# ohsnyt/bzip2-rust

Hardware: AMD Instinct MI355X
Metric: compress MB/s at -9 (900 KB blocks), 1/2/4/8 MI355X; bit-exact vs C bzip2 (higher is better)
Workload: dtype u8; 1 GPU; 1024 MiB per GPU synthetic text at -9 (1194 blocks on this rank), BASELINE configs[2]; raw_bytes_total=1073741824, blocks_rank0=1194, compressed_bytes=323302688

## Files before the change

### bzip2-rust_amd/csrc/bzx_bsort.hip

```cpp
#include <hip/hip_runtime.h>
#include "bzx_host.h"
#include "bzx_wg.h"
#include "bzx_pack.h"

#define BS_NT 1024
#define BS_NW (BS_NT / 64)
#ifndef BS_C
#define BS_C 2048
#endif
#define BS_FW (BS_C / 64)
#define BS_ISO (BS_C / 3)
#ifndef BS_ISO_SHIFT
#define BS_ISO_SHIFT 5
#endif
#ifndef BS_BIN1
#define BS_BIN1 15
#endif
#define BS_BIN2 12
#define BS_NBIN1 (1u << BS_BIN1)
#define BS_TAB_WORDS (BS_NBIN1 + (BS_NBIN1 >> 5))
#define BS_MAX_BK 1024
#ifndef BS_MAX_BIG
#define BS_MAX_BIG 512
#endif
// ... 425 lines not shown
            uint32_t pv[SP_V];
            auto load_tile = [&](uint32_t t0) {
#pragma unroll
                for (uint32_t u = 0; u < SP_V; u++) {
                    const uint32_t i0 = t0 + (u * BS_NT + tid) * 4;
                    hi[u] = lo[u] = 0;
                    pv[u] = 0;
                    if (i0 < n) {
                        uint64_t w2[2];
                        __builtin_memcpy(w2, P + ((i0 * bits) >> 3), 16);
                        hi[u] = w2[0];
                        lo[u] = w2[1];
                        if (i0 >= 1 && i0 + 3 <= n) {
                            __builtin_memcpy(&pv[u], T + i0 - 1, 4);
                        } else {
                            const uint32_t nvalid = n - i0 < 4u ? n - i0 : 4u;
                            for (uint32_t e = 0; e < nvalid; e++) pv[u] |= (uint32_t)T[i0 + e ? i0 + e - 1 : n - 1] << (8 * e);
                        }
                    }
                }
            };
            load_tile(0);
            bzx_lds_barrier();
            uint32_t tpar = 0;
            for (uint32_t t0 = 0; t0 < n; t0 += SP_TILE, tpar ^= 1u) {
                uint32_t *tcnt = tpar ? tcnt1 : tcnt0, *tother = tpar ? tcnt0 : tcnt1;
                uint32_t kr[SP_V * 4], key[SP_V * 4], pvc[SP_V];
#pragma unroll
                for (uint32_t u = 0; u < SP_V; u++) {
                    const uint32_t i0 = t0 + (u * BS_NT + tid) * 4;
                    const uint32_t nvalid = i0 < n ? (n - i0 < 4u ? n - i0 : 4u) : 0u;
                    const uint32_t sh0 = (i0 * bits) & 7u;
                    const uint64_t h = __builtin_bswap64(hi[u]), l = __builtin_bswap64(lo[u]);
                    pvc[u] = pv[u];
#pragma unroll
                    for (uint32_t e = 0; e < 4; e++) {
                        kr[u * 4 + e] = 0xFFFFFFFFu;
                        key[u * 4 + e] = 0;
                        if (e < nvalid) {
                            const uint32_t sh = sh0 + e * bits;
                            const uint64_t w = sh ? (h << sh) | (l >> (64u - sh)) : h;
                            const uint32_t kb = tab16[(uint32_t)(w >> (64 - BS_BIN1))], k = kb & 1023u;
                            key[u * 4 + e] = (uint32_t)((w << (kb >> 10)) >> 32);
                            kr[u * 4 + e] = k | (atomicAdd(&tcnt[k], 1u) << 16);
                        }
                    }
                }
                if (t0 + SP_TILE < n) load_tile(t0 + SP_TILE);
                bzx_lds_barrier();
                {
                    const uint32_t c = tid < nbk ? tcnt[tid] : 0u;
                    const uint32_t incl = bzx_wave_incl_sum(c);
                    uint32_t *wtot = b_scratch + tpar * BS_NW;
                    if (bzx_lane() == 63) wtot[bzx_wave()] = incl;
                    bzx_lds_barrier();
                    uint32_t pre = 0;
                    const uint32_t wv = bzx_wave();
#pragma unroll
                    for (uint32_t i = 0; i < BS_NW; i++) pre += i < wv ? wtot[i] : 0u;
                    const uint32_t ex = pre + incl - c;
                    if (tid < nbk) {
                        tcnt[tid] = ex;
                        tother[tid] = 0;
                        delta[tid] = b_start[tid] + b_cur[tid] - ex;
                        b_cur[tid] += c;
                    }
                }
                bzx_lds_barrier();
#pragma unroll
                for (uint32_t u = 0; u < SP_V; u++)
#pragma unroll
                    for (uint32_t e = 0; e < 4; e++)
                        if (kr[u * 4 + e] != 0xFFFFFFFFu) {
                            const uint32_t k = kr[u * 4 + e] & 0xFFFFu, rel = (u * BS_NT + tid) * 4 + e;
                            stage[tcnt[k] + (kr[u * 4 + e] >> 16)] = ((uint64_t)key[u * 4 + e] << 32) | ((uint64_t)k << 21) | ((uint64_t)rel << 8) |
                                                                     (uint64_t)((pvc[u] >> (8 * e)) & 255u);
                        }
                bzx_lds_barrier();
                const uint32_t tn = n - t0 < SP_TILE ? n - t0 : SP_TILE;
#pragma unroll
                for (uint32_t u = 0; u < SP_TILE / BS_NT; u++) {
                    const uint32_t i = u * BS_NT + tid;
                    if (i < tn) {
                        const uint64_t r = stage[i];
                        const uint32_t k = (uint32_t)(r >> 21) & 1023u, rel = (uint32_t)(r >> 8) & 8191u;
                        rec_a[delta[k] + i] = (r & 0xFFFFFFFF00000000ull) | ((uint64_t)(t0 + rel) << 12) | ((r & 255ull) << 4);
                    }
                }
            }
        }
        __syncthreads();
        DIAG_STAMP(101);
        bool ok = bucket_emit<BS_BIN1>(B, b, j_, nbk, 0, 0, 0, bits, 0, 0);
        DIAG_STAMP(102);

        if (ok) ok = deep_process(B, b, j_, n, bits, P, rec_a, rec_b, 0, 0, BZX_DEEP_LEVELS > 0 ? 0 : -1);
        DIAG_STAMP(103);
        if (!ok) DIAG_COUNT(107, 1);
        if (!ok && tid == 0) block_redo(B, b);
        __syncthreads();
    }
    DIAG_FLUSH();
}

__global__ __launch_bounds__(BS_NT) void bzx_bsplit_deep_kernel(BzxBatch B)
{
    const uint32_t tid = threadIdx.x, lvl = B.deep_lvl;
    const uint32_t listed = B.counters[BZX_CTR_DEEP_CNT + lvl];
    const uint32_t n_items = listed < B.deep_cap ? listed : B.deep_cap;
    if (n_items == 0) return;
    DIAG_T0();
    const BzxDeepItem *list = reinterpret_cast<const BzxDeepItem *>(B.deep_list) + (size_t)(lvl & 1u) * B.deep_cap;
    for (;;) {
        if (tid == 0) b_bcast[0] = atomicAdd(&B.counters[BZX_CTR_DEEP_FETCH + lvl], 1u);
        __syncthreads();
        const uint32_t i = b_bcast[0];
        __syncthreads();
        if (i >= n_items) break;
        const BzxDeepItem d = list[i];
        if (d.cnt == 0) continue;
        const uint32_t b = d.blk;
        if (__atomic_load_n(&B.blk[b].status, __ATOMIC_RELAXED) & BZX_ST_REDO) continue;
        const uint32_t n = B.blk[b].n, bits = d.dbits >> 16;
        const size_t sb = BZX_SLAB(B, b);
        const uint8_t *__restrict__ P = B.pk + sb * BZX_PK_STRIDE;
        uint64_t *__restrict__ rec_a = B.rec_a + sb * BZX_MAX_N;
        uint64_t *__restrict__ rec_b = B.rec_b + sb * BZX_MAX_N;
        if (tid == 0) {
            b_bcast[3] = 1;
            b_bcast[4] = 0;
            b_big[0][0] = d.st;
            b_big[0][1] = d.cnt;
            b_big[0][2] = d.dbits & 0xFFFFu;
        }
        __syncthreads();
        const bool ok = deep_process(B, b, (b - B.blk_first) / B.blk_step, n, bits, P, rec_a, rec_b, 0, 1,
                                     lvl + 1 < BZX_DEEP_LEVELS ? (int)lvl + 1 : -1);
        if (!ok && tid == 0) block_redo(B, b);
        __syncthreads();
    }
    DIAG_FLUSH();
}

#ifndef SK_NT
#define SK_NT 256
#endif
#define SK_NW (SK_NT / 64)
#define BS_E (BS_C / SK_NT)
#define SK_DB 8
#define SK_ND (1u << SK_DB)
static_assert(BS_C % SK_NT == 0 && BS_E >= 1 && BS_E <= 8, "bucket capacity");

__shared__ uint64_t s_x[BS_C];
__shared__ uint64_t s_w[BS_C + 4];
__shared__ uint32_t s_cnt[SK_NW][SK_ND];
__shared__ uint32_t s_dbase[SK_ND];
__shared__ uint32_t s_part[4];
__shared__ uint64_t s_f[BS_FW + 1];
__shared__ uint32_t s_med[BS_C / BS_TINY + 1];
__shared__ uint32_t s_large[BS_C / BS_MED + 1];
__shared__ uint32_t s_rc[2][4];
__shared__ uint32_t s_bc[8];
__shared__ uint32_t s_m[2];
__shared__ uint32_t s_red[SK_NW][4];

__device__ __forceinline__ uint32_t uni(uint32_t v) { return bzx_uni(v); }
__device__ __forceinline__ uint32_t tid_here() { return bzx_tid_here(); }
__device__ __forceinline__ BzxBucket uni(BzxBucket b)
{
    BzxBucket r;
    r.blk = uni(b.blk);
    r.start = uni(b.start);
    r.cnt = uni(b.cnt);
    if (r.cnt >> 31) r.cnt = 0;
    r.dbits = uni(b.dbits);
    return r;
}

__device__ __forceinline__ void wave_rank(uint32_t *wc, uint32_t d, bool valid, uint32_t lane, uint32_t &old, uint32_t &rank)
{
    uint64_t m = __ballot(valid);
    uint32_t plo = (uint32_t)m, phi = (uint32_t)(m >> 32);
#pragma unroll
    for (int b = 0; b < SK_DB; b++) {
        const uint32_t mask = 0u - ((d >> b) & 1u);
        m = __ballot((d >> b) & 1u);
        plo &= ~((uint32_t)m ^ mask);
        phi &= ~((uint32_t)(m >> 32) ^ mask);
    }
    const uint64_t peers = ((uint64_t)phi << 32) | plo;
    rank = (uint32_t)__popcll(peers & ((1ull << lane) - 1ull));
    old = wc[d];
    lds_order();
    if (valid && rank == 0) atomicAdd(&wc[d], (uint32_t)__popcll(peers));
    lds_order();
}

__device__ __attribute__((noinline)) void wg_radix_sort(uint32_t base, uint32_t cnt, int lo, int hi)
{
    uint64_t *A = s_w + base;
    const uint32_t tid = threadIdx.x, lane = bzx_lane(), wave = bzx_wave();
    const uint32_t rows = (cnt + SK_NT - 1) / SK_NT, chunk = rows * 64;
    if (tid == 0) {
        s_bc[5] = 0;
        s_bc[6] = 0;
    }
    __syncthreads();
    {
        const uint64_t a0 = A[0];
        uint64_t d = 0;
#pragma unroll
        for (uint32_t j = 0; j < BS_E; j++) {
            const uint32_t e = wave * chunk + j * 64 + lane;
            if (j < rows && e < cnt) d |= A[e] ^ a0;
        }
#pragma unroll
        for (int s = 32; s > 0; s >>= 1) d |= __shfl_xor(d, s);
        if (lane == 0 && d) {
            atomicOr(&s_bc[5], (uint32_t)d);
            atomicOr(&s_bc[6], (uint32_t)(d >> 32));
        }
    }
    __syncthreads();
    const uint64_t diff = ((uint64_t)s_bc[6] << 32) | s_bc[5];
    uint32_t *wc = s_cnt[wave];
    for (int shift = lo; shift < hi; shift += SK_DB) {
        if (((diff >> shift) & (uint64_t)(SK_ND - 1)) == 0) continue;
#pragma unroll
        for (uint32_t i = 0; i < SK_ND / 64; i++) wc[i * 64 + lane] = 0;
        lds_order();
        uint64_t v[BS_E];
        uint32_t old[BS_E], rk[BS_E];
#pragma unroll
        for (uint32_t j = 0; j < BS_E; j++) {
            const uint32_t e = wave * chunk + j * 64 + lane;
            v[j] = j < rows && e < cnt ? A[e] : 0ull;
        }
#pragma unroll
        for (uint32_t j = 0; j < BS_E; j++) {
            const uint32_t e = wave * chunk + j * 64 + lane;
            wave_rank(wc, (uint32_t)(v[j] >> shift) & (SK_ND - 1), j < rows && e < cnt, lane, old[j], rk[j]);
        }
        __syncthreads();
        {
            constexpr uint32_t SK_DK = SK_ND > SK_NT ? SK_ND / SK_NT : 1u;
            if (tid * SK_DK < SK_ND) {
                uint32_t tot[SK_DK], sum = 0;
#pragma unroll
                for (uint32_t i = 0; i < SK_DK; i++) {
                    uint32_t run = 0;
#pragma unroll
                    for (int w = 0; w < SK_NW; w++) {
                        const uint32_t t = s_cnt[w][tid * SK_DK + i];
                        s_cnt[w][tid * SK_DK + i] = run;
                        run += t;
                    }
                    tot[i] = run;
                    sum += run;
                }
                const uint32_t incl = bzx_wave_incl_sum(sum);
                uint32_t run = incl - sum;
#pragma unroll
                for (uint32_t i = 0; i < SK_DK; i++) {
                    s_dbase[tid * SK_DK + i] = run;
                    run += tot[i];
                }
                if (lane == 63) s_part[wave] = incl;
            }
        }
        __syncthreads();
        const uint32_t p1 = s_part[0], p2 = p1 + s_part[1], p3 = p2 + s_part[2];
#pragma unroll
        for (uint32_t j = 0; j < BS_E; j++) {
            const uint32_t e = wave * chunk + j * 64 + lane;
            if (j < rows && e < cnt) {
                const uint32_t d = (uint32_t)(v[j] >> shift) & (SK_ND - 1);
                const uint32_t q = SK_ND > SK_NT ? 0u : d >> 6;
                A[s_dbase[d] + (q == 0 ? 0u : q == 1 ? p1 : q == 2 ? p2 : p3) + wc[d] + old[j] + rk[j]] = v[j];
            }
        }
        __syncthreads();
    }
}

__device__ __attribute__((noinline)) void wg_radix_sort_opt(uint32_t cnt, int lo, int hi)
{
    uint64_t *A = s_x;
    const uint32_t tid = threadIdx.x, lane = bzx_lane(), wave = bzx_wave();
    const uint32_t rows = (cnt + SK_NT - 1) / SK_NT, chunk = rows * 64;
    __syncthreads();
    uint64_t diff;
    {
        uint32_t o0 = 0, o1 = 0, a0 = ~0u, a1 = ~0u;
#pragma unroll
        for (int w = 0; w < SK_NW; w++) {
            o0 |= s_red[w][0];
            o1 |= s_red[w][1];
            a0 &= s_red[w][2];
            a1 &= s_red[w][3];
        }
        diff = ((uint64_t)(o1 & ~a1) << 32) | (o0 & ~a0);
    }
    uint32_t *wc = s_cnt[wave];
    for (int shift = lo; shift < hi; shift += SK_DB) {
        if (((diff >> shift) & (uint64_t)(SK_ND - 1)) == 0) continue;
#pragma unroll
        for (uint32_t i = 0; i < SK_ND / 64; i++) wc[i * 64 + lane] = 0;
        lds_order();
        uint64_t v[BS_E];
        uint32_t old[BS_E];
#pragma unroll
        for (uint32_t j = 0; j < BS_E; j++) {
            const uint32_t e = wave * chunk + j * 64 + lane;
            v[j] = j < rows && e < cnt ? A[e] : 0ull;
        }
#pragma unroll
        for (uint32_t j = 0; j < BS_E; j++) {
            const uint32_t e = wave * chunk + j * 64 + lane;
            old[j] = bzx_lds_ticket(&wc[(uint32_t)(v[j] >> shift) & (SK_ND - 1)], j < rows && e < cnt);
        }
        __syncthreads();
        {
            static_assert(SK_ND <= SK_NT, "one digit per thread");
            if (tid < SK_ND) {
                uint32_t t[SK_NW], sum = 0;
#pragma unroll
                for (int w = 0; w < SK_NW; w++) {
                    t[w] = s_cnt[w][tid];
                    sum += t[w];
                }
                const uint32_t incl = bzx_wave_incl_sum(sum);
                uint32_t run = incl - sum;
#pragma unroll
                for (int w = 0; w < SK_NW; w++) {
                    s_cnt[w][tid] = run;
                    run += t[w];
                }
                if (lane == 63) s_part[wave] = incl;
            }
        }
        __syncthreads();
        const uint32_t p1 = s_part[0], p2 = p1 + s_part[1], p3 = p2 + s_part[2];
#pragma unroll
        for (uint32_t j = 0; j < BS_E; j++) {
            const uint32_t e = wave * chunk + j * 64 + lane;
            if (j < rows && e < cnt) {
                const uint32_t d = (uint32_t)(v[j] >> shift) & (SK_ND - 1);
                const uint32_t q = d >> 6;
                A[wc[d] + (q == 0 ? 0u : q == 1 ? p1 : q == 2 ? p2 : p3) + old[j]] = v[j];
            }
        }
        __syncthreads();
    }
}

template <bool TICKETS>
__device__ __attribute__((noinline)) void wave_radix_sort(uint32_t base, uint32_t s, int lo, int hi)
{
    constexpr uint32_t ROWS = BS_MED / 64;
    uint64_t *A = s_w + base;
    uint32_t *wc = s_cnt[bzx_wave()];
    const uint32_t lane = bzx_lane();
    const uint32_t rows = (s + 63u) / 64u;
    uint64_t v[ROWS];
    uint64_t diff = 0;
    {
        const uint64_t a0 = A[0];
#pragma unroll
        for (uint32_t j = 0; j < ROWS; j++) {
            const uint32_t e = j * 64 + lane;
            v[j] = e < s ? A[e] : 0ull;
            if (e < s) diff |= v[j] ^ a0;
        }
#pragma unroll
        for (int sh = 32; sh > 0; sh >>= 1) diff |= __shfl_xor(diff, sh);
    }
    for (int shift = lo; shift < hi; shift += SK_DB) {
        if (((diff >> shift) & (uint64_t)(SK_ND - 1)) == 0) continue;
#pragma unroll
        for (uint32_t i = 0; i < SK_ND / 64; i++) wc[i * 64 + lane] = 0;
        lds_order();
        uint32_t old[ROWS], rk[ROWS];
#pragma unroll
        for (uint32_t j = 0; j < ROWS; j++) {
            old[j] = rk[j] = 0;
            if (j < rows) {
                if (TICKETS) old[j] = bzx_lds_ticket(&wc[(uint32_t)(v[j] >> shift) & (SK_ND - 1)], j * 64 + lane < s);
                else wave_rank(wc, (uint32_t)(v[j] >> shift) & (SK_ND - 1), j * 64 + lane < s, lane, old[j], rk[j]);
            }
        }
        {
            uint32_t c[SK_ND / 64], sum = 0;
#pragma unroll
            for (uint32_t i = 0; i < SK_ND / 64; i++) {
                c[i] = wc[(SK_ND / 64) * lane + i];
                sum += c[i];
            }
            uint32_t run = bzx_wave_incl_sum(sum) - sum;
            lds_order();
#pragma unroll
            for (uint32_t i = 0; i < SK_ND / 64; i++) {
                wc[(SK_ND / 64) * lane + i] = run;
                run += c[i];
            }
        }
        lds_order();
#pragma unroll
        for (uint32_t j = 0; j < ROWS; j++)
            if (j * 64 + lane < s) A[wc[(uint32_t)(v[j] >> shift) & (SK_ND - 1)] + old[j] + rk[j]] = v[j];
        lds_order();
#pragma unroll
        for (uint32_t j = 0; j < ROWS; j++) {
            const uint32_t e = j * 64 + lane;
            v[j] = e < s ? A[e] : 0ull;
        }
        lds_order();
    }
}

__device__ __forceinline__ uint32_t fbit(uint32_t p) { return (uint32_t)(s_f[p >> 6] >> (p & 63u)) & 1u; }
__device__ __forceinline__ void fset(uint32_t p) { atomicOr((unsigned long long *)&s_f[p >> 6], 1ull << (p & 63u)); }

__device__ __forceinline__ bool tiny_bounds(uint32_t p, uint32_t &gs, uint32_t &ge)
{
    const uint32_t wi = p >> 6, bi = p & 63u;
    uint64_t w = s_f[wi] & (~0ull >> (63u - bi));
    if (w) {
        gs = wi * 64 + 63u - (uint32_t)__builtin_clzll(w);
    } else {
        if (wi == 0) return false;
        w = s_f[wi - 1];
        if (!w) return false;
        gs = (wi - 1) * 64 + 63u - (uint32_t)__builtin_clzll(w);
    }
    w = bi == 63u ? 0ull : s_f[wi] & (~0ull << (bi + 1u));
    if (w) {
        ge = wi * 64 + (uint32_t)__builtin_ctzll(w);
    } else {
        w = s_f[wi + 1];
        if (!w) return false;
        ge = (wi + 1) * 64 + (uint32_t)__builtin_ctzll(w);
    }
    return ge - gs <= BS_TINY;
}

__device__ __forceinline__ void mark_changes(uint32_t base, uint32_t s, int lo, uint32_t t, uint32_t step)
{
    for (uint32_t e = 1 + t; e < s; e += step)
        if ((s_w[base + e] >> lo) != (s_w[base + e - 1] >> lo)) fset(base + e);
}

__device__ __forceinline__ bool any_big(uint32_t base, uint32_t s, uint32_t t, uint32_t step)
{
    bool big = false;
    for (uint32_t e = t; e < s; e += step) {
        uint32_t gs, ge;
        big |= !tiny_bounds(base + e, gs, ge);
    }
    return big;
}

__device__ __forceinline__ void wave_sort_mark(uint32_t base, uint32_t s, int lo, uint32_t lane)
{
    wave_radix_sort<true>(base, s, lo, 64);
    lds_order();
    uint32_t diff = 0;
    bool bad = false;
    for (uint32_t e = 1 + lane, k = 0; e < s; e += 64, k++) {
        const uint64_t a = s_w[base + e] >> lo, b = s_w[base + e - 1] >> lo;
        bad |= a < b;
        diff |= (uint32_t)(a != b) << k;
    }
    if (__ballot(bad)) {
        wave_radix_sort<false>(base, s, lo, 64);
        mark_changes(base, s, lo, lane, 64);
        return;
    }
    for (uint32_t e = 1 + lane, k = 0; e < s; e += 64, k++)
        if ((diff >> k) & 1u) fset(base + e);
}

__device__ __forceinline__ uint32_t group_start(uint32_t p)
{
    uint32_t wi = p >> 6;
    uint64_t w = s_f[wi] & (~0ull >> (63u - (p & 63u)));
    while (!w) w = s_f[--wi];
    return wi * 64 + 63u - (uint32_t)__builtin_clzll(w);
}

__device__ __forceinline__ uint64_t tied_mask(uint64_t f, uint64_t nx) { return ~(f & ((f >> 1) | (nx << 63))); }

__device__ __forceinline__ void slot_counts_publish(const uint64_t *keep, uint32_t nrow)
{
    const uint32_t lane = bzx_lane(), wave = bzx_wave();
#pragma unroll
    for (uint32_t j = 0; j < BS_E; j++)
        if (j < nrow && lane == 0) s_cnt[0][j * SK_NW + wave] = (uint32_t)__popcll(keep[j]);
}
__device__ __forceinline__ uint32_t slot_counts_sum(uint32_t nrow, uint32_t *before)
{
    const uint32_t wave = bzx_wave();
    uint32_t total = 0;
#pragma unroll
// ... 20 lines not shown
        if ((hmask >> j) & 1u) {
            const uint32_t p = rank_of(j);
            uint32_t wi = p >> 6;
            uint64_t w = (s_f[wi] >> (p & 63u)) >> 1;
            uint32_t e;
            if (w) {
                e = p + 1u + (uint32_t)__builtin_ctzll(w);
            } else {
                do w = s_f[++wi]; while (!w);
                e = wi * 64 + (uint32_t)__builtin_ctzll(w);
            }
            const uint32_t size = e - p;
            if (size > BS_MED) s_large[atomicAdd(&s_rc[par][2], 1u)] = p | (size << 16);
            else if (size > BS_TINY) s_med[atomicAdd(&s_rc[par][1], 1u)] = p | (size << 16);
        }
    }
}

__device__ __forceinline__ void sort_listed_groups(uint32_t par, uint32_t nmed, uint32_t nlarge, uint32_t tid, uint32_t lane)
{
    for (;;) {
        uint32_t k = 0;
        if (lane == 0) k = atomicAdd(&s_rc[par][3], 1u);
        k = __shfl(k, 0);
        if (k >= nmed) break;
        const uint32_t e = s_med[k], gs = e & 0xFFFFu, sz = e >> 16;
        wave_sort_mark(gs, sz, 48, lane);
        lds_order();
        if (__ballot(any_big(gs, sz, lane, 64))) wave_sort_mark(gs, sz, 14, lane);
    }
    for (uint32_t k = 0; k < nlarge; k++) {
        const uint32_t e = s_large[k], gs = e & 0xFFFFu, sz = e >> 16;
        wg_radix_sort(gs, sz, 48, 64);
        mark_changes(gs, sz, 48, tid, SK_NT);
        if (tid == 0) s_bc[2] = 0;
        __syncthreads();
        if (any_big(gs, sz, tid, SK_NT)) s_bc[2] = 1;
        __syncthreads();
        if (s_bc[2]) {
            wg_radix_sort(gs, sz, 14, 64);
            mark_changes(gs, sz, 14, tid, SK_NT);
        }
    }
    __syncthreads();
}

template <typename RankOf>
__device__ __forceinline__ void rank_tiny_groups(uint32_t amask, uint32_t nrow, const RankOf &rank_of, uint32_t (&dst_)[BS_E],
                                                 uint64_t (&my)[BS_E])
{
#pragma unroll
    for (uint32_t j = 0; j < BS_E; j++) {
        dst_[j] = 0xFFFFFFFFu;
        my[j] = 0;
        uint32_t a_ = 0, sz = 0;
        if ((amask >> j) & 1u) {
            const uint32_t p = rank_of(j);
            uint32_t e_;
            if (tiny_bounds(p, a_, e_) && e_ - a_ > 1) {
                sz = e_ - a_;
                my[j] = s_w[p];
            }
        }
        if (j < nrow) {
            uint32_t r = 0, rk = 0;
            const uint64_t myc = my[j] & ~W_POS_MASK;
            for (uint32_t i = 0; i < sz; i += 4) {
                uint64_t wq[4];
#pragma unroll
                for (uint32_t k = 0; k < 4; k++) wq[k] = s_w[a_ + i + k];
#pragma unroll
                for (uint32_t k = 0; k < 4; k++) {
                    const bool in = i + k < sz;
                    r += in && wq[k] < my[j];
                    rk += in && wq[k] < myc;
                }
            }
            if (sz) dst_[j] = (a_ + r) | (r != rk ? 0u : 0x80000000u);
        }
    }
    __syncthreads();
}

__device__ __forceinline__ void place_ranked(const uint32_t (&dst_)[BS_E], const uint64_t (&my)[BS_E])
{
#pragma unroll
    for (uint32_t j = 0; j < BS_E; j++) {
        if (dst_[j] != 0xFFFFFFFFu) {
            const uint32_t q = dst_[j] & 0x7FFFFFFFu;
            s_w[q] = my[j];
            if ((dst_[j] >> 31) && !fbit(q)) fset(q);
        }
    }
    __syncthreads();
}

#define LIST(which, i) (reinterpret_cast<uint16_t *>(s_x)[4u * (i) + 2u + (which)])

template <bool ALL>
__device__ __attribute__((noinline)) void list_tied(uint32_t n, uint32_t from, uint32_t to)
{
    const uint32_t tid = tid_here(), lane = tid & 63u;
    const uint32_t nrow = (n + SK_NT - 1) / SK_NT;
#pragma unroll
    for (uint32_t j = 0; j < BS_E; j++) {
        if (j < nrow) {
            const uint32_t i = j * SK_NT + tid;
            uint32_t p = 0;
            bool t = false;
            if (i < n) {
                p = ALL ? i : (uint32_t)LIST(from, i);
                t = !(fbit(p) && fbit(p + 1));
            }
            const uint64_t mk = __ballot(t);
            if (mk) {
                uint32_t base = 0;
                if (lane == 0) base = atomicAdd(&s_m[to], (uint32_t)__popcll(mk));
                base = bzx_bcast0(base);
                if (t) LIST(to, base + (uint32_t)__popcll(mk & ((1ull << lane) - 1ull))) = (uint16_t)p;
            }
        }
    }
}

__device__ __forceinline__ bool initial_sort(uint32_t cnt)
{
    const uint32_t tid = tid_here(), lane = tid & 63u, wave = tid >> 6;
    uint64_t fm[BS_E];
    wg_radix_sort_opt(cnt, 64 - BS_KEYBITS, 64);
    int bad = 0;
#pragma unroll
    for (uint32_t j = 0; j < BS_E; j++) {
        const uint32_t p = j * SK_NT + tid;
        s_w[p] = p;
        const uint64_t kp = s_x[p] >> (64 - BS_KEYBITS), kq = p ? s_x[p - 1] >> (64 - BS_KEYBITS) : 0ull;
        const bool f = p >= cnt || p == 0 || kp != kq;
        bad |= p < cnt && p > 0 && kp < kq;
        fm[j] = __ballot(f);
        if (lane == 0) s_f[j * SK_NW + wave] = fm[j];
    }
    if (tid == 0) s_f[BS_FW] = ~0ull;
    if (__syncthreads_or(bad)) return false;
#pragma unroll
    for (uint32_t j = 0; j < BS_E; j++) {
        const uint64_t mk = tied_mask(fm[j], s_f[j * SK_NW + wave + 1]);
        if (mk) {
            uint32_t base = 0;
            if (lane == 0) base = atomicAdd(&s_m[0], (uint32_t)__popcll(mk));
            base = bzx_bcast0(base);
            if ((mk >> lane) & 1ull) LIST(0, base + (uint32_t)__popcll(mk & ((1ull << lane) - 1ull))) = (uint16_t)(j * SK_NT + tid);
        }
    }
    return true;
}

#ifndef SK_WAVES_PER_SIMD
#define SK_WAVES_PER_SIMD 4
#endif
#ifdef BZX_HIP_EMU
#define BS_LOAD_REC(p) (*(p))
#else
#define BS_LOAD_REC(p) __builtin_nontemporal_load(p)
#endif
__device__ __forceinline__ void bsort_body(const BzxBatch &B)
{
    const uint32_t tid0 = threadIdx.x;
    if (B.bsort_mode == 1 && B.counters[BZX_CTR_RESUME] == 0) return;
    DIAG_T0();
    const uint32_t G = gridDim.x >> 3;
    const uint32_t cap8 = B.bk_cap >> 3, lx = blockIdx.x & 7u;
    const uint32_t n_lx = B.counters[BZX_CTR_BK_LIST0 + lx] < cap8 ? B.counters[BZX_CTR_BK_LIST0 + lx] : cap8;
    const uint32_t n_items = lx * cap8 + n_lx;
    uint32_t idx = lx * cap8 + (blockIdx.x >> 3);
    BzxBucket it = {0, 0, 0, 0}, nit = {0, 0, 0, 0};
    if (idx < n_items) it = uni(B.bk_list[idx]);
    if (idx + G < n_items) nit = uni(B.bk_list[idx + G]);
    uint64_t nxt[BS_E];
    uint32_t n_cur = 0, st_cur = 0;
    if (it.cnt) {
        const uint64_t *__restrict__ src = ((it.start >> 31) ? B.rec_b : B.rec_a) + BZX_SLAB(B, it.blk) * BZX_MAX_N +
                                           (it.start & 0x7fffffffu);
#pragma unroll
        for (uint32_t j = 0; j < BS_E; j++) nxt[j] = j * SK_NT + tid0 < it.cnt ? BS_LOAD_REC(src + j * SK_NT + tid0) : ~0ull;
        n_cur = uni(B.blk[it.blk].n);
        st_cur = uni(__atomic_load_n(&B.blk[it.blk].status, __ATOMIC_RELAXED));
    }
    for (; idx < n_items; idx += G) {
        BzxBucket nit2 = {0, 0, 0, 0};
        if (idx + 2 * G < n_items) nit2 = B.bk_list[idx + 2 * G];
        uint32_t tid = tid_here(), lane = tid & 63u, wave = tid >> 6;
        const uint32_t b = it.blk, cnt = it.cnt;
        const uint32_t start = it.start & 0x7fffffffu, bits = it.dbits >> 16, depth0 = it.dbits & 0xFFFFu;
        const uint8_t *__restrict__ P = B.pk + BZX_SLAB(B, b) * BZX_PK_STRIDE;
        const uint32_t nbits = n_cur * bits;
        const bool skip = cnt == 0 || (cnt >> 31) || (st_cur & BZX_ST_REDO) || (B.bsort_mode == 1 && !(st_cur & BZX_ST_RESUME));
        DIAG_STAMP(64);
        if (!skip) {
            uint32_t o0 = 0, o1 = 0, a0 = ~0u, a1 = ~0u;
#pragma unroll
            for (uint32_t j = 0; j < BS_E; j++) {
                s_x[j * SK_NT + tid] = nxt[j];
                if (j * SK_NT + tid < cnt) {
                    o0 |= (uint32_t)nxt[j];
                    o1 |= (uint32_t)(nxt[j] >> 32);
                    a0 &= (uint32_t)nxt[j];
                    a1 &= (uint32_t)(nxt[j] >> 32);
                }
            }
            o0 = bzx_wave_incl_or(o0);
            o1 = bzx_wave_incl_or(o1);
            a0 = bzx_wave_incl_and(a0);
            a1 = bzx_wave_incl_and(a1);
            if (lane == 63) {
                s_red[wave][0] = o0;
                s_red[wave][1] = o1;
                s_red[wave][2] = a0;
                s_red[wave][3] = a1;
            }
        }
        uint32_t n_nx = 0, st_nx = 0;
#define PREFETCH_NEXT()                                                                                                   \
        if (nit.cnt) {                                                                                                    \
            const uint64_t *__restrict__ src = ((nit.start >> 31) ? B.rec_b : B.rec_a) + BZX_SLAB(B, nit.blk) * BZX_MAX_N + \
                                               (nit.start & 0x7fffffffu);                                                 \
            const uint32_t tp_ = tid_here();                                                                              \
            _Pragma("unroll") for (uint32_t j = 0; j < BS_E; j++) nxt[j] = j * SK_NT + tp_ < nit.cnt ? BS_LOAD_REC(src + j * SK_NT + tp_) : ~0ull; \
            n_nx = B.blk[nit.blk].n;                                             \
            st_nx = __atomic_load_n(&B.blk[nit.blk].status, __ATOMIC_RELAXED);                                            \
        }
        if (skip) {
            PREFETCH_NEXT();
            it = nit;
            nit = uni(nit2);
            n_cur = uni(n_nx);
            st_cur = uni(st_nx);
            continue;
        }
        if (tid == 0) s_rc[0][0] = s_rc[0][1] = s_rc[0][2] = s_rc[0][3] = s_m[0] = s_m[1] = 0;
        DIAG_STAMP(65);
        if (!initial_sort(cnt)) {
            if (tid == 0) {
                atomicAdd(&B.counters[BZX_CTR_STAT0 + 15], 1u);
                block_redo(B, b);
            }
            PREFETCH_NEXT();
            __syncthreads();
            it = nit;
            nit = uni(nit2);
            n_cur = uni(n_nx);
            st_cur = uni(st_nx);
            continue;
        }
        DIAG_STAMP(67);

        uint32_t dcur = depth0 + BS_KEYBITS;
        bool fail = false;
        uint32_t lpar = 0;
        __syncthreads();
        DIAG_STAMP(73);
        for (uint32_t round = 0;; round++) {
            tid = tid_here();
            lane = tid & 63u;
            wave = tid >> 6;
            const uint32_t par = round & 1u;
            const uint32_t m = uni(s_m[lpar]);
            if (m == 0) break;
            if (!(round < BS_ROUNDS && dcur < nbits)) {
                DIAG_COUNT(round >= BS_ROUNDS ? 84 : 85, 1);
                fail = true;
                break;
            }
            DIAG_COUNT(80, 1);
            DIAG_COUNT(88, m);
            const uint32_t nrow = (m + SK_NT - 1) / SK_NT;
            uint32_t amask = 0, hmask = 0;
            uint32_t pq[BS_E], xa[BS_E];
#pragma unroll
            for (uint32_t j = 0; j < BS_E; j++) {
                pq[j] = 0;
                xa[j] = 0;
                if (j < nrow) {
                    const uint32_t i = j * SK_NT + tid;
                    if (i < m) {
                        const uint32_t p = LIST(lpar, i);
                        amask |= 1u << j;
                        hmask |= fbit(p) << j;
                        pq[j] = p | ((uint32_t)(s_w[p] & W_POS_MASK) << 16);
                    }
                }
            }
#pragma unroll
            for (uint32_t j = 0; j < BS_E; j++) {
                if ((amask >> j) & 1u) {
                    uint32_t x = REC_IDX(s_x[pq[j] >> 16]) * bits + dcur;
                    if (x >= nbits) x -= nbits;
                    xa[j] = x;
                }
            }
            uint64_t g[BS_E];
#pragma unroll
            for (uint32_t j = 0; j < BS_E; j++) g[j] = ((amask >> j) & 1u) ? pk_window_bit(P, xa[j]) : 0ull;
            const auto rank_of = [&](uint32_t j) { return pq[j] & 0xFFFFu; };
            list_big_groups(hmask, par, rank_of);
#pragma unroll
            for (uint32_t j = 0; j < BS_E; j++)
                if ((amask >> j) & 1u) s_w[pq[j] & 0xFFFFu] = (g[j] & ~W_POS_MASK) | (uint64_t)(pq[j] >> 16);
            if (tid == 0) {
                s_rc[par ^ 1u][0] = s_rc[par ^ 1u][1] = s_rc[par ^ 1u][2] = s_rc[par ^ 1u][3] = 0;
                s_m[lpar ^ 1u] = 0;
            }
            __syncthreads();
            DIAG_STAMP(68);
            const uint32_t nmed = s_rc[par][1], nlarge = s_rc[par][2];
            if (nmed | nlarge) {
                DIAG_COUNT(86, nmed);
                DIAG_COUNT(87, nlarge);
                sort_listed_groups(par, nmed, nlarge, tid, lane);
                DIAG_STAMP(69);
            }
            tid = tid_here();
            lane = tid & 63u;
            wave = tid >> 6;
            uint32_t dst_[BS_E];
            uint64_t my[BS_E];
            rank_tiny_groups(amask, nrow, rank_of, dst_, my);
            DIAG_STAMP(70);
            place_ranked(dst_, my);
            DIAG_STAMP(71);
            list_tied<false>(m, lpar, lpar ^ 1u);
            __syncthreads();
            DIAG_STAMP(73);
            lpar ^= 1u;
            dcur += 50;
        }
        PREFETCH_NEXT();
        tid = tid_here();
        if (fail || B.bsort_mode == 1) {
            uint64_t *__restrict__ sax = B.rec_a + BZX_SLAB(B, b) * BZX_MAX_N + start;
            const uint32_t rk = uni(B.blk[b].n_selectors);
            uint32_t *__restrict__ isa0 = rank_array(B, rk, 0), *__restrict__ isa1 = rank_array(B, rk, 1);
#pragma unroll
            for (uint32_t j = 0; j < BS_E; j++) {
                const uint32_t p = j * SK_NT + tid;
                if (p < cnt) {
                    const uint32_t rot = REC_IDX(s_x[(uint32_t)(s_w[p] & W_POS_MASK)]);
                    const uint32_t f0 = fbit(p);
                    sax[p] = (uint64_t)rot | ((uint64_t)f0 << 32);
                    if (isa0) {
                        const uint32_t head = f0 ? p : group_start(p);
                        isa0[rot] = start + head;
                        if (f0 && fbit(p + 1)) isa1[rot] = start + head;
                    }
                }
            }
            if (fail) {
                uint32_t *__restrict__ cl = reinterpret_cast<uint32_t *>(B.rec_b + BZX_SLAB(B, b) * BZX_MAX_N + start);
                uint64_t mk[BS_E];
                lane = tid & 63u;
                wave = tid >> 6;
#pragma unroll
                for (uint32_t j = 0; j < BS_E; j++) mk[j] = tied_mask(s_f[j * SK_NW + wave], s_f[j * SK_NW + wave + 1]);
                slot_counts_publish(mk, BS_E);
                __syncthreads();
                uint32_t before[BS_E];
                const uint32_t total = slot_counts_sum(BS_E, before);
#pragma unroll
                for (uint32_t j = 0; j < BS_E; j++) {
                    if ((mk[j] >> lane) & 1ull) {
                        const uint32_t p = j * SK_NT + tid;
                        const uint32_t rot = REC_IDX(s_x[(uint32_t)(s_w[p] & W_POS_MASK)]);
                        cl[before[j] + (uint32_t)__popcll(mk[j] & ((1ull << lane) - 1ull))] = p | (fbit(p) << 11) | (rot << 12);
                    }
                }
                if (tid == 0) {
                    atomicMin(&B.blk[b].n_mtf, dcur / bits);
                    B.bk_list[idx].cnt = cnt | 0x80000000u;
                    const uint32_t ri = atomicAdd(&B.counters[BZX_CTR_RK_ITEMS], 1u);
                    B.rk_list[ri] = idx;
                    B.rk_list[B.bk_cap + ri] = total;
                    atomicAdd(&B.counters[BZX_CTR_RK_OPEN], 1u);
                    atomicAdd(&B.blk[b].n_groups, 1u);
                    if ((atomicOr(&B.blk[b].status, BZX_ST_RESUME) & BZX_ST_RESUME) == 0)
                        B.resume_list[atomicAdd(&B.counters[BZX_CTR_RESUME], 1u)] = b;
                }
            }
        }
        {
            constexpr uint32_t OUT_E = 8;
            uint8_t *__restrict__ L = B.bwt + BZX_SLAB(B, b) * BZX_BLK_STRIDE + start;
            const uint32_t p0 = tid * OUT_E;
            if (p0 < cnt) {
                uint64_t w8[OUT_E];
#pragma unroll
                for (uint32_t k = 0; k < OUT_E; k++) w8[k] = s_w[p0 + k];
                uint64_t bytes = 0;
#pragma unroll
                for (uint32_t k = 0; k < OUT_E; k++) {
                    const uint32_t r = reinterpret_cast<const uint32_t *>(s_x)[2u * (uint32_t)(w8[k] & W_POS_MASK)];
                    bytes |= (uint64_t)REC_PREV(r) << (8 * k);
                    if (p0 + k < cnt && REC_IDX(r) == 0) B.blk[b].orig_ptr = start + p0 + k;
                }
                if (p0 + OUT_E <= cnt) {
                    __builtin_memcpy(L + p0, &bytes, 8);
                } else {
                    for (uint32_t k = 0; p0 + k < cnt; k++) L[p0 + k] = (uint8_t)(bytes >> (8 * k));
                }
            }
            DIAG_COUNT(83, 1);
        }
        __syncthreads();
        DIAG_STAMP(72);
        it = nit;
        nit = uni(nit2);
        n_cur = uni(n_nx);
        st_cur = uni(st_nx);
    }
    DIAG_FLUSH();
}

__global__ __launch_bounds__(SK_NT, SK_WAVES_PER_SIMD) void bzx_bsort_kernel(BzxBatch B) { bsort_body(B); }
__global__ __launch_bounds__(SK_NT, SK_WAVES_PER_SIMD) void bzx_bfill_kernel(BzxBatch B) { bsort_body(B); }

#define RK_CHUNK 16
struct RkMeta {
    uint32_t bi, T, blk, start, cnt, n, rk, h0;
};
__shared__ RkMeta s_meta[RK_CHUNK];

__device__ __forceinline__ uint32_t rk_fetch_chunk(const BzxBatch &B, uint32_t n_items, uint32_t &open)
{
    __shared__ uint32_t s_fetch[2];
    __syncthreads();
    if (threadIdx.x < 64) {
        uint32_t base = 0;
        if (threadIdx.x == 0) base = atomicAdd(&B.counters[B.rk_fetch], (uint32_t)RK_CHUNK);
        base = __shfl(base, 0);
        const uint32_t i = base + threadIdx.x;
        bool op = false;
        if (threadIdx.x < RK_CHUNK && i < n_items) {
            RkMeta m;
            m.bi = B.rk_list[i];
            m.T = B.rk_list[B.bk_cap + i];
            const BzxBucket it = B.bk_list[m.bi];
            op = !(it.dbits >> 31);
            m.blk = it.blk;
            m.start = it.start & 0x7fffffffu;
            m.cnt = it.cnt & 0x7fffffffu;
            m.n = B.blk[it.blk].n;
            m.rk = B.blk[it.blk].n_selectors;
            m.h0 = B.blk[it.blk].n_mtf;
            s_meta[threadIdx.x] = m;
        }
        const uint64_t m = __ballot(op);
        if (threadIdx.x == 0) {
            s_fetch[0] = base;
            s_fetch[1] = (uint32_t)m;
        }
    }
    __syncthreads();
    open = s_fetch[1];
    return s_fetch[0];
}

__shared__ uint32_t s_stall[2 * BS_FW];

__device__ __forceinline__ void rank_round_wave(const BzxBatch &B, uint32_t i)
{
    const uint32_t lane = bzx_lane(), wave = bzx_wave();
    const RkMeta &mt = s_meta[i & (RK_CHUNK - 1)];
    const uint32_t bi = bzx_bcast0(mt.bi);
    const uint32_t T = bzx_bcast0(mt.T);
    const uint32_t b = bzx_bcast0(mt.blk), start = bzx_bcast0(mt.start);
    const uint32_t rk = bzx_bcast0(mt.rk);
    uint32_t *__restrict__ isa_r = rank_array(B, rk, B.rk_h_shift & 1u);
    uint32_t *__restrict__ isa_w = rank_array(B, rk, (B.rk_h_shift & 1u) ^ 1u);
    const uint32_t n = bzx_bcast0(mt.n);
    const uint64_t h64 = (uint64_t)bzx_bcast0(mt.h0) * B.rk_h_mul;
    if (!isa_r || h64 >= n) return;
    const uint32_t h = (uint32_t)h64;
    uint32_t *__restrict__ cl = reinterpret_cast<uint32_t *>(B.rec_b + BZX_SLAB(B, b) * BZX_MAX_N + start);
    uint64_t *wk = s_w + wave * 64;
    uint32_t *wr = reinterpret_cast<uint32_t *>(s_x + wave * 64);
    const uint32_t ent = lane < T ? cl[lane] : (1u << 11);
    const uint32_t rot = ent >> 12, pc = ent & 2047u;
    const uint64_t F = __ballot(lane >= T || ((ent >> 11) & 1u));
    const bool f1 = lane == 63 ? true : (F >> (lane + 1)) & 1ull;
    const bool single = lane < T && ((F >> lane) & 1ull) && f1;
    const bool tied = lane < T && !single;
    if (single) isa_w[rot] = start + pc;
    uint32_t x = rot + h;
    if (x >= n) x -= n;
    uint32_t x2 = x + h;
    if (x2 >= n) x2 -= n;
    const uint32_t ahead = tied ? isa_r[x] : 0u, ahead2 = tied ? isa_r[x2] : 0u;
    const uint32_t gs = 63u - (uint32_t)__builtin_clzll((F & (~0ull >> (63u - lane))) | 1ull);
    const uint64_t above = lane == 63 ? 0ull : F >> (lane + 1);
    const uint32_t ge = above ? lane + 1u + (uint32_t)__builtin_ctzll(above) : 64u;
    const uint64_t C = __ballot((ahead | ahead2) >> 31);
    const bool stall = tied && (C & (~0ull >> (64u - ge)) & (~0ull << gs)) != 0;
    const uint64_t key = tied ? (stall ? 0ull : ((uint64_t)ahead << 28) | ((uint64_t)ahead2 << 8)) | lane : 0ull;
    lds_order();
    wk[lane] = key;
    lds_order();
    uint32_t r = 0, eq = 0;
    const uint32_t sz = tied ? ge - gs : 0u;
    for (uint32_t k = 0; __ballot(k < sz); k++) {
        if (k < sz) {
            const uint64_t o = wk[gs + k];
            const bool lt = o < key;
            r += lt;
            eq += lt && (o >> 8) == (key >> 8);
        }
    }
    lds_order();
    if (tied) wr[2 * (gs + r)] = rot | (eq ? 0u : 1u << 20);
    lds_order();
    const uint32_t nv = tied ? wr[2 * lane] : 0u;
    const uint32_t rot_n = nv & 0xFFFFFu;
    const uint64_t Fn = __ballot(!tied || ((F >> lane) & 1ull) || ((nv >> 20) & 1u));
    const uint32_t hc = 63u - (uint32_t)__builtin_clzll((Fn & (~0ull >> (63u - lane))) | 1ull);
    const uint32_t p_head = (uint32_t)__shfl((int)pc, (int)hc);
    const bool f0n = (Fn >> lane) & 1ull, f1n = lane == 63 ? true : (Fn >> (lane + 1)) & 1ull;
    uint32_t out = 0;
    if (stall) {
        isa_r[rot_n] = isa_w[rot_n] = (start + p_head) | RK_COARSE;
        uint64_t *__restrict__ sax = B.rec_a + BZX_SLAB(B, b) * BZX_MAX_N + start;
        sax[pc] = (uint64_t)rot_n | ((uint64_t)f0n << 32);
    } else if (tied) {
        isa_w[rot_n] = start + p_head;
        out = pc | ((uint32_t)f0n << 11) | (rot_n << 12);
        uint64_t *__restrict__ sax = B.rec_a + BZX_SLAB(B, b) * BZX_MAX_N + start;
        if (f0n && f1n) {
            const uint8_t *__restrict__ Tx = BZX_BLOCK_PTR(B, B.blk[b]);
            uint8_t *__restrict__ L = B.bwt + BZX_SLAB(B, b) * BZX_BLK_STRIDE + start;
            L[pc] = Tx[rot_n ? rot_n - 1 : n - 1];
            sax[pc] = (uint64_t)rot_n | (1ull << 32);
            if (rot_n == 0) B.blk[b].orig_ptr = start + pc;
        } else if (B.rk_last) {
            sax[pc] = (uint64_t)rot_n | ((uint64_t)f0n << 32);
        }
    }
    const uint64_t keep = __ballot(tied && !stall);
    if (tied && !stall) cl[(uint32_t)__popcll(keep & ((1ull << lane) - 1ull))] = out;
    if (lane == 0) {
        const uint32_t Tn = (uint32_t)__popcll(keep);
        B.rk_list[B.bk_cap + i] = Tn;
        if (C) atomicAdd(&B.blk[b].n_groups, 1u);
        if (Tn == 0) {
            B.bk_list[bi].dbits |= 0x80000000u;
            atomicSub(&B.counters[BZX_CTR_RK_OPEN], 1u);
            if (atomicSub(&B.blk[b].n_groups, 1u) == 1u) atomicAnd(&B.blk[b].status, ~BZX_ST_RESUME);
        }
    }
// ... 459 lines not shown
```

Measured before the change: 28920 MB/s.

## Streamline bucket sort: per-wave digit scan, single-wave tail rounds, rotated output reads

In the workgroup radix sort, every wave now computes its own exclusive digit offsets from vectorized uint4 reads of all waves' counts and writes them to a per-wave table. This removes one workgroup barrier and the partition-select arithmetic from each pass. When 64 or fewer unresolved tie groups remain, a new noinline wave_rounds routine lets wave 0 finish the refinement rounds alone, using wave-level ordering instead of workgroup barriers. The BWT output loop rotates each thread's read order to spread LDS bank accesses, and the counter initialization is split across several threads. The per-wave table reuses s_w as scratch, which relies on s_w not being live during the radix passes, and the single-wave path leaves the other waves idle.

New measurement: 29800 MB/s, median of 6. 1.03x the previous value.

```diff
diff --git a/bzip2-rust_amd/csrc/bzx_bsort.hip b/bzip2-rust_amd/csrc/bzx_bsort.hip
--- a/bzip2-rust_amd/csrc/bzx_bsort.hip
+++ b/bzip2-rust_amd/csrc/bzx_bsort.hip
@@ -601,8 +601,8 @@
 static_assert(BS_C % SK_NT == 0 && BS_E >= 1 && BS_E <= 8, "bucket capacity");
 
 __shared__ uint64_t s_x[BS_C];
-__shared__ uint64_t s_w[BS_C + 4];
-__shared__ uint32_t s_cnt[SK_NW][SK_ND];
+__shared__ __attribute__((aligned(16))) uint64_t s_w[BS_C + 4];
+__shared__ __attribute__((aligned(16))) uint32_t s_cnt[SK_NW][SK_ND];
 __shared__ uint32_t s_dbase[SK_ND];
 __shared__ uint32_t s_part[4];
 __shared__ uint64_t s_f[BS_FW + 1];
@@ -735,7 +735,7 @@
 __device__ __attribute__((noinline)) void wg_radix_sort_opt(uint32_t cnt, int lo, int hi)
 {
     uint64_t *A = s_x;
-    const uint32_t tid = threadIdx.x, lane = bzx_lane(), wave = bzx_wave();
+    const uint32_t lane = bzx_lane(), wave = bzx_wave();
     const uint32_t rows = (cnt + SK_NT - 1) / SK_NT, chunk = rows * 64;
     __syncthreads();
     uint64_t diff;
@@ -751,6 +751,7 @@
         diff = ((uint64_t)(o1 & ~a1) << 32) | (o0 & ~a0);
     }
     uint32_t *wc = s_cnt[wave];
+    uint32_t *wb = reinterpret_cast<uint32_t *>(s_w) + wave * SK_ND;
     for (int shift = lo; shift < hi; shift += SK_DB) {
         if (((diff >> shift) & (uint64_t)(SK_ND - 1)) == 0) continue;
 #pragma unroll
@@ -770,34 +771,38 @@
         }
         __syncthreads();
         {
-            static_assert(SK_ND <= SK_NT, "one digit per thread");
-            if (tid < SK_ND) {
-                uint32_t t[SK_NW], sum = 0;
-#pragma unroll
-                for (int w = 0; w < SK_NW; w++) {
-                    t[w] = s_cnt[w][tid];
-                    sum += t[w];
-                }
-                const uint32_t incl = bzx_wave_incl_sum(sum);
-                uint32_t run = incl - sum;
-#pragma unroll
-                for (int w = 0; w < SK_NW; w++) {
-                    s_cnt[w][tid] = run;
-                    run += t[w];
-                }
-                if (lane == 63) s_part[wave] = incl;
-            }
-        }
-        __syncthreads();
-        const uint32_t p1 = s_part[0], p2 = p1 + s_part[1], p3 = p2 + s_part[2];
+            static_assert(SK_ND == 4 * 64, "four digits per lane");
+            uint32_t mine[4], tot[4], sum = 0;
+#pragma unroll
+            for (uint32_t i = 0; i < 4; i++) mine[i] = tot[i] = 0;
+#pragma unroll
+            for (uint32_t w = 0; w < SK_NW; w++) {
+                const uint4 c = *reinterpret_cast<const uint4 *>(&s_cnt[w][4 * lane]);
+                const uint32_t cc[4] = {c.x, c.y, c.z, c.w};
+#pragma unroll
+                for (uint32_t i = 0; i < 4; i++) {
+                    if (w < wave) mine[i] += cc[i];
+                    tot[i] += cc[i];
+                }
+            }
+#pragma unroll
+            for (uint32_t i = 0; i < 4; i++) sum += tot[i];
+            uint32_t run = bzx_wave_incl_sum(sum) - sum;
+            uint4 o;
+            o.x = run + mine[0];
+            run += tot[0];
+            o.y = run + mine[1];
+            run += tot[1];
+            o.z = run + mine[2];
+            run += tot[2];
+            o.w = run + mine[3];
+            *reinterpret_cast<uint4 *>(&wb[4 * lane]) = o;
+        }
+        lds_order();
 #pragma unroll
         for (uint32_t j = 0; j < BS_E; j++) {
             const uint32_t e = wave * chunk + j * 64 + lane;
-            if (j < rows && e < cnt) {
-                const uint32_t d = (uint32_t)(v[j] >> shift) & (SK_ND - 1);
-                const uint32_t q = d >> 6;
-                A[wc[d] + (q == 0 ? 0u : q == 1 ? p1 : q == 2 ? p2 : p3) + old[j]] = v[j];
-            }
+            if (j < rows && e < cnt) A[wb[(uint32_t)(v[j] >> shift) & (SK_ND - 1)] + old[j]] = v[j];
         }
         __syncthreads();
     }
@@ -1124,6 +1129,54 @@
         }
     }
     return true;
+}
+
+__device__ __attribute__((noinline)) uint32_t wave_rounds(const uint8_t *__restrict__ P, uint32_t bits, uint32_t nbits, uint32_t m,
+                                                          uint32_t lpar, uint32_t round, uint32_t dcur)
+{
+    const uint32_t lane = bzx_lane();
+    for (;; round++) {
+        if (m == 0) return dcur;
+        if (!(round < BS_ROUNDS && dcur < nbits)) return dcur | 0x80000000u;
+        const bool has = lane < m;
+        uint32_t p = 0, gs = 0, ge = 0;
+        uint64_t my = 0;
+        if (has) {
+            p = LIST(lpar, lane);
+            const uint32_t pos = (uint32_t)(s_w[p] & W_POS_MASK);
+            uint32_t x = REC_IDX(s_x[pos]) * bits + dcur;
+            if (x >= nbits) x -= nbits;
+            my = (pk_window_bit(P, x) & ~W_POS_MASK) | pos;
+            tiny_bounds(p, gs, ge);
+        }
+        lds_order();
+        if (has) s_w[p] = my;
+        lds_order();
+        uint32_t r = 0, rk = 0;
+        const uint64_t myc = my & ~W_POS_MASK;
+        const uint32_t sz = ge - gs;
+        for (uint32_t i = 0; __ballot(i < sz); i++) {
+            if (i < sz) {
+                const uint64_t o = s_w[gs + i];
+                r += o < my;
+                rk += o < myc;
+            }
+        }
+        lds_order();
+        if (has) {
+            const uint32_t q = gs + r;
+            s_w[q] = my;
+            if (r == rk && !fbit(q)) fset(q);
+        }
+        lds_order();
+        const bool t = has && !(fbit(p) && fbit(p + 1));
+        const uint64_t mk = __ballot(t);
+        if (t) LIST(lpar ^ 1u, (uint32_t)__popcll(mk & ((1ull << lane) - 1ull))) = (uint16_t)p;
+        lds_order();
+        m = (uint32_t)__popcll(mk);
+        lpar ^= 1u;
+        dcur += 50;
+    }
 }
 
 #ifndef SK_WAVES_PER_SIMD
@@ -1208,7 +1261,8 @@
             st_cur = uni(st_nx);
             continue;
         }
-        if (tid == 0) s_rc[0][0] = s_rc[0][1] = s_rc[0][2] = s_rc[0][3] = s_m[0] = s_m[1] = 0;
+        if (tid < 4) s_rc[0][tid] = 0;
+        if (tid < 2) s_m[tid] = 0;
         DIAG_STAMP(65);
         if (!initial_sort(cnt)) {
             if (tid == 0) {
@@ -1237,6 +1291,19 @@
             const uint32_t par = round & 1u;
             const uint32_t m = uni(s_m[lpar]);
             if (m == 0) break;
+            if (m <= 64) {
+                DIAG_COUNT(89, 1);
+                if (wave == 0) {
+                    dcur = wave_rounds(P, bits, nbits, m, lpar, round, dcur);
+                    if (lane == 0) s_bc[3] = dcur;
+                }
+                __syncthreads();
+                dcur = uni(s_bc[3]);
+                fail = dcur >> 31;
+                dcur &= 0x7FFFFFFFu;
+                DIAG_STAMP(70);
+                break;
+            }
             if (!(round < BS_ROUNDS && dcur < nbits)) {
                 DIAG_COUNT(round >= BS_ROUNDS ? 84 : 85, 1);
                 fail = true;
@@ -1362,15 +1429,17 @@
             uint8_t *__restrict__ L = B.bwt + BZX_SLAB(B, b) * BZX_BLK_STRIDE + start;
             const uint32_t p0 = tid * OUT_E;
             if (p0 < cnt) {
-                uint64_t w8[OUT_E];
-#pragma unroll
-                for (uint32_t k = 0; k < OUT_E; k++) w8[k] = s_w[p0 + k];
+                const uint32_t rot = tid >> 2;
+                uint32_t pos[OUT_E];
+#pragma unroll
+                for (uint32_t k = 0; k < OUT_E; k++) pos[k] = (uint32_t)(s_w[p0 + ((k + rot) & (OUT_E - 1))] & W_POS_MASK);
                 uint64_t bytes = 0;
 #pragma unroll
                 for (uint32_t k = 0; k < OUT_E; k++) {
-                    const uint32_t r = reinterpret_cast<const uint32_t *>(s_x)[2u * (uint32_t)(w8[k] & W_POS_MASK)];
-                    bytes |= (uint64_t)REC_PREV(r) << (8 * k);
-                    if (p0 + k < cnt && REC_IDX(r) == 0) B.blk[b].orig_ptr = start + p0 + k;
+                    const uint32_t kk = (k + rot) & (OUT_E - 1);
+                    const uint32_t r = reinterpret_cast<const uint32_t *>(s_x)[2u * pos[k]];
+                    bytes |= (uint64_t)REC_PREV(r) << (8 * kk);
+                    if (p0 + kk < cnt && REC_IDX(r) == 0) B.blk[b].orig_ptr = start + p0 + kk;
                 }
                 if (p0 + OUT_E <= cnt) {
                     __builtin_memcpy(L + p0, &bytes, 8);
```
